# yeyupiaoling/MASR

Hardware: AMD Instinct MI355X
Metric: audio-seconds/sec (RTF^-1), conformer_streaming_fbank b32x10s, PCM->fbank->encoder->ctc_greedy->text (higher is better)
Workload: dtype f32; 1 GPU; configs[1]: conformer.yml streaming fbank, batch=32 synthetic 16 kHz 10 s utterances per GPU, ctc_greedy, random-init weights V=4233; global_batch=32, parallelism=dp1, world_size_observed=1, backend=none

## Files before the change

masr_amd/csrc/common.h:

```cpp
#pragma once
#include <hip/hip_runtime.h>
#include <stdint.h>

#include "lm_scorer.h"

#ifndef MASR_EXPERIMENTS
#define MASR_EXPERIMENTS 0
#endif

typedef float f32x4 __attribute__((ext_vector_type(4)));
typedef float f32x16 __attribute__((ext_vector_type(16)));

namespace masr {

struct LdsAttr {
    size_t granted[32] = {};
};
void ensure_dynamic_lds(const void* fn, size_t bytes, LdsAttr& st);
void note_launch_error(const char* what, hipError_t e);

#ifdef __HIPCC__
struct SeqRow {
    int b, t;
};
__device__ __forceinline__ SeqRow seq_row(int b0, int t0, int T, int lr) {
    SeqRow r{b0, t0 + lr};
    while (r.t >= T) {
        r.t -= T;
        ++r.b;
    }
    return r;
}

__device__ __forceinline__ float wave_sum_dpp(float v) {
#define MASR_DPP_F(x, ctrl, rows) \
    __builtin_bit_cast(float, __builtin_amdgcn_update_dpp(0, __builtin_bit_cast(int, (x)), (ctrl), (rows), 0xf, false))
    v += MASR_DPP_F(v, 0x111, 0xf);
    v += MASR_DPP_F(v, 0x112, 0xf);
    v += MASR_DPP_F(v, 0x114, 0xf);
    v += MASR_DPP_F(v, 0x118, 0xf);
    v += MASR_DPP_F(v, 0x142, 0xa);
    v += MASR_DPP_F(v, 0x143, 0xc);
#undef MASR_DPP_F
    return __builtin_bit_cast(float, __builtin_amdgcn_readlane(__builtin_bit_cast(int, v), 63));
}
#endif


enum GemmAct { ACT_NONE = 0, ACT_RELU = 1, ACT_SILU = 2 };
enum GemmAMode { A_PLAIN = 0, A_CONV2 = 1 };
enum GemmEpi { EPI_STD = 0, EPI_GLU = 1, EPI_SPLITK = 2 };

struct GemmArgs {
    const float* A;
    const float* W;
    const float* bias;
    float* C;
    const float* R;
    const int* lens;
    int M, N, K;
    int lda, ldc, ldr;
    int act;
    float alpha;
    int mask_tp;
    int bias_after_alpha;
    int T1, F1, T2, F2, Cc;
    int nsplit, ksplit;
    int skip_rps, skip_div;
};

void launch_gemm(const GemmArgs& a, int amode, int epi, hipStream_t s);
void set_conv2_mid_fill(int pct);
void set_gemm_waves(int n);
void launch_gemm_splitk(const GemmArgs& a, float* partial, int nsplit, hipStream_t s, int amode = A_PLAIN);
#if MASR_EXPERIMENTS
bool launch_gemm_bf16x3(const GemmArgs& a, int amode, hipStream_t s);
void set_gemm_bf16x3_waves(int n);
size_t ffn_x3_packed_elems(int dff);
void set_ffn_x3_rotation(int on);
void launch_pack_ffn_x3(const float* w1, const float* w2, unsigned short* p1, unsigned short* p2, int dff, hipStream_t s);
bool launch_ffn_x3(float* x, const float* lnw, const float* lnb, const unsigned short* p1, const float* b1,
                   const unsigned short* p2, const float* b2, int M, int dff, float eps, float scale, hipStream_t s);
#else
inline bool launch_gemm_bf16x3(const GemmArgs&, int, hipStream_t) { return false; }
inline void set_gemm_bf16x3_waves(int) {}
inline size_t ffn_x3_packed_elems(int) { return 0; }
inline void set_ffn_x3_rotation(int) {}
inline void launch_pack_ffn_x3(const float*, const float*, unsigned short*, unsigned short*, int, hipStream_t) {}
inline bool launch_ffn_x3(float*, const float*, const float*, const unsigned short*, const float*, const unsigned short*, const float*,
                          int, int, float, float, hipStream_t) { return false; }
#endif

void launch_layernorm(const float* x, const float* w, const float* b, float* y, int M, float eps,
                      int seq_t, int pad, const int* lens, hipStream_t s);
void set_conv1_nt(int on);
void launch_conv1(const float* feats, const float* mean, const float* istd, const float* w9c, const float* bias,
                  float* out, int B, int T, int F, int C, hipStream_t s);
void launch_dwconv_ln_silu(const float* g, const float* wkc, const float* bias, const float* lnw, const float* lnb,
                           float* out, int nseq, int Tq, int ktaps, float eps, hipStream_t s, const float* gconst = nullptr);
void launch_glu_const(const float* bias512, float* out256, hipStream_t s);
void launch_queue_spin(long long ticks, hipStream_t s);
void launch_queue_nop(hipStream_t s);
void launch_dwconv_bn_silu(const float* g, const float* wkc, const float* bias, const float* scale, const float* shift,
                           float* out, int nseq, int Tq, int ktaps, hipStream_t s, const float* gconst = nullptr);
void launch_dwconv_stride2_ln_silu(const float* g, const float* wkc, const float* bias, const float* lnw,
                                   const float* lnb, float* out, int nseq, int Tin, int ktaps, float eps, hipStream_t s);
void launch_avgpool2(const float* x, float* out, int B, int T, hipStream_t s);
void launch_time_reduce_dw(const float* x, const float* w5c, const float* bias, const int* lens, float* out, int B, int T,
                           int mstride, hipStream_t s);
void launch_recover_add(const float* saved, const float* y, float* x, int B, int T, int L, hipStream_t s);
void launch_softmax_argmax(float* logits, int M, int V, int ldv, int write_probs, int* idx, float* maxp, hipStream_t s);
void launch_ctc_collapse(const int* idx, const float* maxp, const int* nframes, int B, int Tp, int blank,
                         int* tokens, int* ntok, float* score, hipStream_t s);
struct PoolSeg {
    long src, dst;
    int n, pad_;
};
void launch_ctc_collapse_hist(const int* idx, const float* maxp, const int* nframes, const int* in_rows, int ld_in, int B, int Tp,
                              int blank, int* rows, hipStream_t s);
void launch_copy_segments(const float* src, float* dst, const float* src2, float* dst2, const PoolSeg* seg, int nseg,
                          int max_rows, int width, hipStream_t s);
void launch_ctc_collapse_rows(const int* idx, const float* maxp, const int* nframes, int B, int Tp, int blank, int* rows,
                              hipStream_t s);
void launch_topk_prune(const float* probs, int M, int V, int top_n, float cutoff_prob, int* out_idx, float* out_logp,
                       int* out_cnt, int blank, float* out_blank_lp, hipStream_t s);
void launch_argmax_rows(const float* probs, int M, int V, int* idx, float* maxp, hipStream_t s);
void launch_frame_counts(const int* nsamp, int B, int* nfr, int* nenc, int halve, hipStream_t s);
void launch_export_att(const float* cache, float* out, int L, int H, int cap, int t, int dk, hipStream_t s, int rate = 1,
                       int shift = 0);
struct PlaneCopy { const float* src_k; const float* src_v; float* dst_k; float* dst_v; };
void launch_kv_append_planar(const PlaneCopy* pc, int n, int Tq, hipStream_t s);
void launch_export_cnn_layer(const float* cache, float* out, int used, int total, int d, hipStream_t s);
void launch_export_att_planar(const float* kplane, const float* vplane, float* out, int H, int t, int dk, hipStream_t s);
void launch_affine_rows(const float* x, const float* w, const float* b, float* y, int M, int seq_t, int pad, hipStream_t s);
void launch_export_cnn(const float* cache, float* out, int L, int pad, int d, hipStream_t s);

struct AttSeq;
enum RowGemmPro { RG_PRO_PLAIN = 0, RG_PRO_LN = 1, RG_PRO_LN_PAD = 2, RG_PRO_AFFINE = 3,
                  RG_PRO_HIST = 4, RG_PRO_DWCONV = 5 };
enum RowGemmEpi { RG_EPI_STORE = 0, RG_EPI_RESID = 1, RG_EPI_GLU = 2, RG_EPI_CTC = 3, RG_EPI_CHAIN = 4 };
struct RowGemmArgs {
    const float* A;
    const float* lnw;
    const float* lnb;
    const float* W;
    const float* Wp;
    const float* bias;
    float* C;
    const float* R;
    float* R2;
    const int* lens;
    int* out_idx;
    float* out_maxp;
    int M, N;
    int lda, ldc, ldr;
    float eps, alpha;
// ... 220 lines not shown
```

masr_amd/csrc/engine.hip:

```cpp
#include <math.h>
#include <stdio.h>
#include <stdlib.h>
#include <string.h>

#include <map>
#include <mutex>
#include <string>
#include <vector>

#include "../../include/masr_hip.h"
#include "common.h"

using namespace masr;
namespace masr {
int lm_device_view(masr_lm* lm, LmView* out);
bool lm_word_based(const masr_lm* lm);
}
extern "C" const char* masr_lm_last_error(void);

static thread_local std::string g_err;
static int fail(const std::string& m) {
    g_err = m;
    return 1;
}
// ... 147 lines not shown
    int kin;
};

struct HostTensor {
    std::vector<float> v;
    std::vector<int64_t> shape;
};

struct Stream {
    bool open = false;
    int offset = 0;
    int offset_r = 0;
    int cap = 0;
    int history = -1;
    int cache_t1 = 0;
    int first_half = 0;
    DevBuf att;
    DevBuf cnn;
    DevBuf cnn2;
};

struct GBeam {
    bool open = false, started = false;
    int beam = 0, blank = 0, cap = 0;
    DevBuf pool, state;
    masr_lm* lm = nullptr;
    float alpha = 0.f, beta = 0.f;
};

enum ProfKind { PROF_NONE = 0, PROF_GEMM = 1, PROF_FFN1 = 2, PROF_CONV2 = 3, PROF_ATT = 4, PROF_FBANK = 5,
                PROF_FFN_TAIL = 6, PROF_FFN_HEAD = 7 };

}

struct EngineWs {
    DevBuf gx, rnn_out, hstate, cstate, ds2_lens;
    PinnedStage stage;
    DevBuf qplanes, attp, cnnptrs, ffpart;
    DevBuf fb_scratch;
    DevBuf x1, x2, x, ln, hid, qkv, att, lnpad, glu, dwo, logits, feats, enc, idx, maxp, attseq, gain, nframes, lens, xsave,
        xred, xh;
    void release_all() {
        for (DevBuf* b : {&gx, &rnn_out, &hstate, &cstate, &ds2_lens, &qplanes, &attp, &cnnptrs, &ffpart, &fb_scratch, &x1, &x2, &x,
                          &ln, &hid, &qkv, &att, &lnpad, &glu, &dwo, &logits, &feats, &enc, &idx, &maxp, &attseq, &gain, &nframes,
                          &lens, &xsave, &xred, &xh})
            b->release();
        stage.release();
    }
};

static int clear_sync(void* p, int value, size_t n) {
    HIPCHK(hipMemset(p, value, n));
    HIPCHK(hipStreamSynchronize(nullptr));
    return 0;
}

struct masr_engine : EngineWs {
    masr_config cfg;
    EngineWs parked[MASR_LANES];
    int lane = 0;
    hipEvent_t pack_ev = nullptr;
    void* pack_stream = nullptr;
    bool pack_pending = false;
    bool finalized = false;
    std::map<std::string, HostTensor> host;
    std::vector<void*> owned;
    float *cmvn_mean = nullptr, *cmvn_istd = nullptr, *conv1_w = nullptr, *conv1_b = nullptr, *conv2_w = nullptr,
          *conv2_b = nullptr, *embed_w = nullptr, *embed_b = nullptr, *after_w = nullptr, *after_b = nullptr,
          *ctc_w = nullptr, *ctc_b = nullptr, *pe = nullptr;
    std::vector<LayerW> layers;
    std::vector<SqLayerW> sq_layers;
    std::vector<Ds2LayerW> ds2_layers;
    std::vector<GBeam> gbeams;
    DevBuf beam_pool, beam_state;
    std::map<void*, std::pair<DevBuf, DevBuf>> beam_ws;
    std::map<void*, DevBuf> ms_ws;
    int skip_padding = 7;
    void* beam_first_stream = nullptr;
    bool beam_first_set = false;
    std::map<const float*, std::pair<DevBuf, DevBuf>> ffn_packed;
    std::map<const float*, std::pair<DevBuf, DevBuf>> ffn_dual_packed;
    std::map<const float*, std::pair<DevBuf, DevBuf>> x3_packed;
    std::map<const float*, std::pair<DevBuf, DevBuf>> ffn16_packed;
    long long* beam_prof = nullptr;
    float *preln_w = nullptr, *preln_b = nullptr, *tr_dw_w = nullptr, *tr_dw_b = nullptr, *tr_pw_w = nullptr,
          *tr_pw_b = nullptr, *rec_w = nullptr, *rec_b = nullptr;
    int reduce_idx = -1, recover_idx = -1;
    int stride_idx = -1, n_group_layers = 0, group_size = 3;
    bool conv_bn = false;
    float *window = nullptr, *melwt = nullptr, *tw512 = nullptr, *twr4 = nullptr;
    FbankTables fbank_tables() const { return FbankTables{window, melwt, tw512, twr4, mel_lo}; }
    int* mel_lo = nullptr;
    float *dct = nullptr, *lifter = nullptr;
    int dct_ceps = 0;
    double *lin_win = nullptr, *lin_tw = nullptr;
    double lin_scale = 0.0;
    std::vector<Stream> streams;
    int prof_kind = 0;
    int prof_stride = 1, prof_seen = 0;
    std::vector<std::pair<hipEvent_t, hipEvent_t>> prof_events;
    size_t prof_used = 0;
    double prof_flops = 0.0;
};

namespace {

template <class T>
int upload(masr_engine* e, const std::vector<T>& v, T** out) {
    void* p = nullptr;
    HIPCHK(hipMalloc(&p, std::max<size_t>(v.size(), 1) * sizeof(T)));
    HIPCHK(hipMemcpy(p, v.data(), v.size() * sizeof(T), hipMemcpyHostToDevice));
    e->owned.push_back(p);
    *out = reinterpret_cast<T*>(p);
    return 0;
}

int get(masr_engine* e, const std::string& name, std::vector<int64_t> shape, const HostTensor** out) {
    auto it = e->host.find(name);
    if (it == e->host.end()) return fail("missing tensor: " + name);
    int64_t want = 1, have = 1;
    for (auto s : shape) want *= s;
    for (auto s : it->second.shape) have *= s;
    if (want != have)
        return fail("tensor " + name + ": expected " + std::to_string(want) + " elements, got " + std::to_string(have));
    *out = &it->second;
    return 0;
}

int up(masr_engine* e, const std::string& name, std::vector<int64_t> shape, float** out) {
    const HostTensor* t;
    CHK(get(e, name, shape, &t));
    return upload(e, t->v, out);
}

struct ProfScope {
    masr_engine* e;
    hipStream_t s;
    bool on;
    ProfScope(masr_engine* e_, hipStream_t s_, int kind, double flops) : e(e_), s(s_) {
        on = e->prof_kind != 0 && (e->prof_kind == kind || (e->prof_kind == PROF_GEMM && (kind == PROF_FFN1 || kind == PROF_CONV2 || kind == PROF_FFN_TAIL || kind == PROF_FFN_HEAD)));
        if (on && e->prof_stride > 1) on = (e->prof_seen++ % e->prof_stride) == 0;
        if (!on) return;
        if (e->prof_used == e->prof_events.size()) {
            hipEvent_t a, b;
            hipEventCreate(&a);
            hipEventCreate(&b);
            e->prof_events.push_back({a, b});
        }
        hipEventRecord(e->prof_events[e->prof_used].first, s);
        e->prof_flops += flops;
    }
    ~ProfScope() {
        if (!on) return;
        hipEventRecord(e->prof_events[e->prof_used].second, s);
        e->prof_used++;
    }
};

struct CallGuard {
    masr_engine* e;
    hipStream_t s;
    size_t n0;
    static size_t packed_count(const masr_engine* e) {
        return e->ffn_packed.size() + e->ffn_dual_packed.size() + e->x3_packed.size() + e->ffn16_packed.size();
    }
    CallGuard(masr_engine* e_, hipStream_t s_) : e(e_), s(s_), n0(packed_count(e_)) {
        if (!e->pack_pending) return;
        if (hipEventQuery(e->pack_ev) == hipSuccess) {
            e->pack_pending = false;
        } else {
            (void)hipGetLastError();
            if ((void*)s != e->pack_stream) (void)hipStreamWaitEvent(s, e->pack_ev, 0);
        }
    }
    ~CallGuard() {
        if (packed_count(e) == n0) return;
        if (!e->pack_ev && hipEventCreateWithFlags(&e->pack_ev, hipEventDisableTiming) != hipSuccess) return;
        if (hipEventRecord(e->pack_ev, s) == hipSuccess) {
            e->pack_stream = (void*)s;
            e->pack_pending = true;
        }
    }
};

static int g_ffn_dual = 0;
static int g_ffn_packed = 2;
static int g_ffn16 = 1;
static int g_bf16x3 = 0;

void gemm(masr_engine* e, hipStream_t s, const float* A, int lda, const float* W, const float* bias, float* C, int ldc,
          int M, int N, int K, int act, float alpha, const float* R, int ldr, int kind = PROF_GEMM,
          const int* lens = nullptr, int mask_tp = 0) {
    GemmArgs a{};
    a.A = A; a.W = W; a.bias = bias; a.C = C; a.R = R; a.lens = lens;
    a.M = M; a.N = N; a.K = K; a.lda = lda; a.ldc = ldc; a.ldr = ldr;
    a.act = act; a.alpha = alpha; a.mask_tp = mask_tp;
    ProfScope ps(e, s, kind, 2.0 * M * (double)N * K);
    if (g_bf16x3 && launch_gemm_bf16x3(a, A_PLAIN, s)) return;
    launch_gemm(a, A_PLAIN, EPI_STD, s);
}

static int g_rowgemm_packed = 1;
const float* packed_rows_of(masr_engine* e, const float* W, int N, hipStream_t s) {
    auto it = e->ffn_packed.find(W);
    if (it == e->ffn_packed.end()) {
        const int Np = (N + 255) / 256 * 256;
        std::pair<DevBuf, DevBuf> pk;
        if (pk.first.ensure((size_t)Np * 256 * sizeof(float))) return nullptr;
        launch_pack_rows_pc(W, pk.first.as<float>(), Np, s, N);
        it = e->ffn_packed.emplace(W, pk).first;
    }
    return it->second.first.as<float>();
}

int packed_ffn_of(masr_engine* e, const float* w1, const float* w2, hipStream_t s, const float** p1, const float** p2) {
    const int d = e->cfg.d_model;
    auto it = e->ffn_packed.find(w1);
    if (it == e->ffn_packed.end()) {
        std::pair<DevBuf, DevBuf> pk;
        CHK(pk.first.ensure((size_t)e->cfg.d_ff * d * sizeof(float)));
        CHK(pk.second.ensure((size_t)e->cfg.d_ff * d * sizeof(float)));
        launch_pack_ffn_pc(w1, w2, pk.first.as<float>(), pk.second.as<float>(), e->cfg.d_ff, s);
        it = e->ffn_packed.emplace(w1, pk).first;
    }
    *p1 = it->second.first.as<float>();
    *p2 = it->second.second.as<float>();
    return 0;
}
static bool sqz_stage_supported(const masr_engine* e) {
    const int K = e->cfg.cnn_kernel;
    return e->cfg.d_model == 256 && e->cfg.d_ff % 128 == 0 && e->cfg.d_ff >= 256 && (K == 31 || K == 15);
}

void rowgemm(masr_engine* e, hipStream_t s, int pro, int epi, const float* A, int lda, const float* lnw,
             const float* lnb, const float* W, const float* bias, float* C, int ldc, int M, int N, const float* R,
             int ldr, float alpha, const int* lens, int mask_tp, int seq_t, int pad, int* out_idx, float* out_maxp,
             int kind = PROF_GEMM, int mstride = 4, int out_seq_t = 0, int out_pad_l = 0, int out_pad_tot = 0,
             int plane_cols = 0, long plane_stride = 0, int a_seq_t = 0, int a_seq_stride = 0, const AttSeq* kv_seqs = nullptr,
             int kv_tq = 0) {
    RowGemmArgs a{};
    a.A = A; a.lda = lda; a.lnw = lnw; a.lnb = lnb; a.W = W; a.bias = bias; a.C = C; a.ldc = ldc; a.M = M; a.N = N;
    a.R = R; a.ldr = ldr; a.alpha = alpha; a.lens = lens; a.mask_tp = mask_tp; a.seq_t = seq_t; a.pad = pad;
    a.out_idx = out_idx; a.out_maxp = out_maxp; a.eps = 1e-5f; a.mstride = mstride;
    a.out_seq_t = out_seq_t; a.out_pad_l = out_pad_l; a.out_pad_tot = out_pad_tot;
    a.plane_cols = plane_cols; a.plane_stride = plane_stride; a.a_seq_t = a_seq_t; a.a_seq_stride = a_seq_stride;
    a.kv_seqs = kv_seqs; a.kv_tq = kv_tq;
    if (g_rowgemm_packed && M >= 112 * 32 && pro != RG_PRO_HIST && pro != RG_PRO_DWCONV && (epi == RG_EPI_CTC || N % 256 == 0))
        a.Wp = packed_rows_of(e, W, N, s);
    ProfScope ps(e, s, kind, 2.0 * M * (double)N * 256);
    launch_rowgemm(a, pro, epi, s);
}

}

namespace {
int build_fbank_tables(masr_engine* e) {
    {
        std::vector<float> win(400), tw512(2 * 257), melw((size_t)80 * 257, 0.f);
        std::vector<int> lo(80), hi(80);
        for (int i = 0; i < 400; ++i) {
            const double hann = 0.5 - 0.5 * cos(2.0 * M_PI * i / 399.0);
            win[i] = (float)pow(hann, 0.85);
        }
        for (int k = 0; k <= 256; ++k) {
            tw512[2 * k] = (float)cos(-2.0 * M_PI * k / 512.0);
            tw512[2 * k + 1] = (float)sin(-2.0 * M_PI * k / 512.0);
        }
        const double mel_low = 1127.0 * log(1.0 + 20.0 / 700.0), mel_high = 1127.0 * log(1.0 + 8000.0 / 700.0);
        const float delta = (float)((mel_high - mel_low) / 81.0), mlow = (float)mel_low;
        for (int m = 0; m < 80; ++m) {
// ... 117 lines not shown
    if (cfg->model_kind < 0 || cfg->model_kind > 3)
        return fail("model_kind must be 0 (conformer), 1 (squeezeformer, non-streaming), 2 (efficient_conformer) or 3 (deepspeech2)");
    if (cfg->n_mels < 7 || cfg->n_mels > 512) return fail("input feature size (n_mels) must be in [7, 512]");
    if (cfg->model_kind == 3) {
        if (cfg->d_model != 1024) return fail("deepspeech2: the LSTM step kernel is specialised for rnn_size=1024");
        if (cfg->num_blocks <= 0) return fail("deepspeech2: num_rnn_layers must be positive");
    } else if (cfg->d_model != 256 || cfg->heads != 4) {
        return fail("kernels are specialised for d_model=256, heads=4");
    } else if (cfg->d_ff % 128) {
        return fail("unsupported d_ff");
    }
    if (cfg->model_kind == 3) {
    } else if (cfg->model_kind == 0 || cfg->model_kind == 2) {
        if (cfg->cnn_kernel != 15) return fail("conformer: cnn_module_kernel must be 15");
    } else {
        if (cfg->cnn_kernel != 31) return fail("squeezeformer: cnn_module_kernel must be 31");
    }
    int ndev = 0;
    HIPCHK(hipGetDeviceCount(&ndev));
    if (ndev <= 0) return fail("no HIP device");
    HIPCHK(hipSetDevice(cfg->device_id));
    {
        SideStreams* ss = nullptr;
        if (side_streams_of(cfg->device_id, &ss)) return 1;
    }
    masr_engine* e = new masr_engine();
    e->cfg = *cfg;
    if (e->cfg.max_pos <= 0) e->cfg.max_pos = 5000;
    e->reduce_idx = cfg->model_kind == 1 ? cfg->reserved[0] : -1;
    e->conv_bn = cfg->model_kind == 0 && cfg->reserved[0] == 1;
    e->recover_idx = cfg->model_kind == 1 ? cfg->reserved[1] : -1;
    if (cfg->model_kind == 2) {
        e->stride_idx = cfg->reserved[0];
        e->n_group_layers = cfg->reserved[1];
        e->group_size = cfg->reserved[2];
        if (e->group_size != 3) { delete e; return fail("efficient_conformer: group_size must be 3"); }
    }
    if (build_fbank_tables(e)) {
        masr_destroy(e);
        return 1;
    }
    *out = e;
    return 0;
}

void masr_destroy(masr_engine* e) {
    if (!e) return;
    for (void* p : e->owned) (void)hipFree(p);
    e->release_all();
    for (auto& w : e->parked) w.release_all();
    e->beam_pool.release();
    e->beam_state.release();
    if (e->pack_ev) (void)hipEventDestroy(e->pack_ev);
    for (auto& s : e->streams) {
        s.att.release();
        s.cnn.release();
        s.cnn2.release();
    }
    for (auto& g : e->gbeams) {
        g.pool.release();
        g.state.release();
    }
    for (auto& kv : e->beam_ws) {
        kv.second.first.release();
        kv.second.second.release();
    }
    for (auto& kv : e->ms_ws) kv.second.release();
    for (auto& kv : e->x3_packed) {
        kv.second.first.release();
        kv.second.second.release();
    }
    for (auto& kv : e->ffn_packed) {
        kv.second.first.release();
        kv.second.second.release();
    }
    for (auto& kv : e->ffn_dual_packed) {
        kv.second.first.release();
        kv.second.second.release();
    }
    for (auto& kv : e->ffn16_packed) {
        kv.second.first.release();
        kv.second.second.release();
    }
    for (auto& ev : e->prof_events) {
        (void)hipEventDestroy(ev.first);
        (void)hipEventDestroy(ev.second);
    }
    delete e;
}

static void drop_packed_weights(masr_engine* e) {
    if (e->ffn_packed.empty() && e->ffn_dual_packed.empty() && e->x3_packed.empty() && e->ffn16_packed.empty()) return;
    (void)hipSetDevice(e->cfg.device_id);
    (void)hipDeviceSynchronize();
    for (auto* m : {&e->ffn_packed, &e->ffn_dual_packed, &e->x3_packed, &e->ffn16_packed}) {
        for (auto& kv : *m) {
            kv.second.first.release();
            kv.second.second.release();
        }
        m->clear();
    }
}

int masr_load_tensor(masr_engine* e, const char* name, const float* host, const int64_t* shape, int32_t ndim) {
    if (!e || !name || !host) return fail("null argument");
    std::string n(name);
    if (n.rfind("encoder.", 0) != 0 && n.rfind("ctc.", 0) != 0 && n.rfind("decoder.ctc_lo.", 0) != 0 && n != "__pos_table__")
        return 0;
    drop_packed_weights(e);
    HostTensor t;
    int64_t cnt = 1;
    for (int i = 0; i < ndim; ++i) {
        t.shape.push_back(shape[i]);
        cnt *= shape[i];
    }
    t.v.assign(host, host + cnt);
    e->host[n] = std::move(t);
    e->finalized = false;
    return 0;
}

static int finalize_squeezeformer(masr_engine* e, hipStream_t s);
static int finalize_ds2(masr_engine* e);
static int enc_dim(const masr_engine* e) {
    return e->cfg.model_kind == 3 ? e->cfg.d_model * (e->cfg.causal ? 1 : 2) : e->cfg.d_model;
}
static int layer_kernel(const masr_engine* e, int i) {
    return (e->cfg.model_kind == 2 && e->stride_idx >= 0 && i > e->stride_idx) ? e->cfg.cnn_kernel / 2 : e->cfg.cnn_kernel;
}
static bool layer_grouped(const masr_engine* e, int i) { return e->cfg.model_kind == 2 && i < e->n_group_layers; }

int masr_finalize(masr_engine* e, void* stream) {
    if (!e) return fail("null engine");
    if (e->cfg.model_kind == 1) return finalize_squeezeformer(e, (hipStream_t)stream);
    if (e->cfg.model_kind == 3) return finalize_ds2(e);
    hipStream_t s = (hipStream_t)stream;
    HIPCHK(hipSetDevice(e->cfg.device_id));
    const int d = e->cfg.d_model, dff = e->cfg.d_ff, L = e->cfg.num_blocks, V = e->cfg.vocab_size, F = e->cfg.n_mels;
    const int F1 = (F - 1) / 2, F2 = (F1 - 1) / 2, K = e->cfg.cnn_kernel, H = e->cfg.heads, dk = d / H;
    const HostTensor* t;
    CHK(up(e, "encoder.global_cmvn.mean", {F}, &e->cmvn_mean));
    CHK(up(e, "encoder.global_cmvn.istd", {F}, &e->cmvn_istd));
    {
        CHK(get(e, "encoder.embed.conv.0.weight", {d, 1, 3, 3}, &t));
        std::vector<float> w(9 * d);
        for (int c = 0; c < d; ++c)
            for (int k = 0; k < 9; ++k) w[k * d + c] = t->v[c * 9 + k];
        CHK(upload(e, w, &e->conv1_w));
        CHK(up(e, "encoder.embed.conv.0.bias", {d}, &e->conv1_b));
    }
    {
        CHK(get(e, "encoder.embed.conv.2.weight", {d, d, 3, 3}, &t));
        std::vector<float> w((size_t)d * 9 * d);
        for (int co = 0; co < d; ++co)
            for (int ci = 0; ci < d; ++ci)
                for (int k = 0; k < 9; ++k)
                    w[(size_t)co * 9 * d + (size_t)(ci / 32) * 9 * 32 + k * 32 + ci % 32] = t->v[((size_t)co * d + ci) * 9 + k];
        CHK(upload(e, w, &e->conv2_w));
        CHK(up(e, "encoder.embed.conv.2.bias", {d}, &e->conv2_b));
    }
    {
        CHK(get(e, "encoder.embed.out.0.weight", {d, (int64_t)d * F2}, &t));
        std::vector<float> w((size_t)d * d * F2);
        for (int o = 0; o < d; ++o)
            for (int c = 0; c < d; ++c)
                for (int f = 0; f < F2; ++f) w[(size_t)o * d * F2 + f * d + c] = t->v[(size_t)o * d * F2 + c * F2 + f];
        CHK(upload(e, w, &e->embed_w));
        CHK(up(e, "encoder.embed.out.0.bias", {d}, &e->embed_b));
    }
    {
        auto it = e->host.find("__pos_table__");
        if (it != e->host.end()) {
            if ((int64_t)it->second.v.size() != (int64_t)e->cfg.max_pos * d) return fail("__pos_table__ has wrong size");
            CHK(upload(e, it->second.v, &e->pe));
        } else {
            std::vector<float> pe((size_t)e->cfg.max_pos * d);
            for (int i = 0; i < d; i += 2) {
                const float div = expf((float)i * (float)(-(log(10000.0) / d)));
// ... 259 lines not shown
            auto it = e->ffn16_packed.find(W);
            if (it == e->ffn16_packed.end()) {
                std::pair<DevBuf, DevBuf> pk;
                CHK(pk.first.ensure((size_t)N * d * sizeof(float)));
                launch_pack_rows16(W, pk.first.as<float>(), N, s);
                it = e->ffn16_packed.emplace(W, pk).first;
            }
            *out = it->second.first.as<float>();
            return 0;
        };
        auto it = e->ffn16_packed.find(w1);
        if (it == e->ffn16_packed.end()) {
            std::pair<DevBuf, DevBuf> pk;
            CHK(pk.first.ensure((size_t)dff * d * sizeof(float)));
            CHK(pk.second.ensure((size_t)dff * d * sizeof(float)));
            launch_pack_ffn16(w1, w2, pk.first.as<float>(), pk.second.as<float>(), dff, s);
            it = e->ffn16_packed.emplace(w1, pk).first;
        }
        if (want_tail) {
            ptail = *tail;
            CHK(p16(tail->W, tail->N, &ptail.W));
        }
        if (want_head) {
            phead = *head;
            CHK(p16(head->W, d, &phead.W));
        }
        const int done = launch_ffn16(e->x.as<float>(), lnw, lnb, it->second.first.as<float>(), b1, it->second.second.as<float>(), b2, M,
                                      dff, 1e-5f, scale, s, want_tail ? &ptail : nullptr, want_head ? &phead : nullptr);
        if (done < 0) return fail("ffn(): the 16-row FFN kernel rejected the launch");
        if (want_head && done != 4) return fail("ffn(): head stage was not launched");
        if (tail_done) *tail_done = done == 2;
        if (post_y) launch_layernorm(e->x.as<float>(), post_w, post_b, post_y, M, 1e-5f, 0, 0, nullptr, s);
        return 0;
    }
    if (packed && want_tail && tail->N % 256 == 0) {
        ptail = *tail;
        CHK(packed_rows(tail->W, tail->N, &ptail.W));
        tail = &ptail;
    }
    if (packed && want_head) {
        phead = *head;
        CHK(packed_rows(head->W, d, &phead.W));
        if (split_head) {
            CHK(e->xh.ensure((size_t)M * d * sizeof(float)));
            phead.xout = e->xh.as<float>();
        }
        head = &phead;
    }
    const int done = launch_ffn_fused(e->x.as<float>(), lnw, lnb, kw1, b1, kw2, b2, M, dff, 1e-5f, scale, affine,
                                      nsplit > 1 ? e->ffpart.as<float>() : nullptr, nsplit, s, post_y ? &post : nullptr,
                                      want_tail ? tail : nullptr, want_head ? head : nullptr, packed);
    if (done < 0) return fail("ffn(): launch rejected");
    if (want_head && !(done & 4)) return fail("ffn(): head stage was not launched");
    if (tail_done) *tail_done = done == 2;
    if (post_y && !(done & 1)) launch_layernorm(e->x.as<float>(), post_w, post_b, post_y, M, 1e-5f, 0, 0, nullptr, s);
    return 0;
}

static int g_hot_weights = 0;
static int g_embed_split = 1;
int embed(masr_engine* e, hipStream_t s, const float* feats, int nseq, int T, int* Tq_out, const int* skip_lens = nullptr) {
    const int d = e->cfg.d_model, F = e->cfg.n_mels, F1 = (F - 1) / 2, F2 = (F1 - 1) / 2;
    const int T1 = (T - 1) / 2, Tq = (T1 - 1) / 2;
    if (T < 7 || Tq <= 0) return fail("input too short for Conv2dSubsampling4 (need >= 7 frames)");
    const int M = nseq * Tq;
    CHK(e->x1.ensure((size_t)nseq * T1 * F1 * d * sizeof(float)));
    CHK(e->x2.ensure((size_t)M * F2 * d * sizeof(float)));
    CHK(e->x.ensure((size_t)M * d * sizeof(float)));
    launch_conv1(feats, e->cmvn_mean, e->cmvn_istd, e->conv1_w, e->conv1_b, e->x1.as<float>(), nseq, T, F, d, s);
    {
        GemmArgs a{};
        a.A = e->x1.as<float>(); a.W = e->conv2_w; a.bias = e->conv2_b; a.C = e->x2.as<float>();
        a.M = M * F2; a.N = d; a.K = 9 * d; a.ldc = d; a.act = ACT_RELU; a.alpha = 1.f;
        a.T1 = T1; a.F1 = F1; a.T2 = Tq; a.F2 = F2; a.Cc = d;
        if (skip_lens) { a.lens = skip_lens; a.skip_rps = Tq * F2; a.skip_div = F2; }
        ProfScope ps(e, s, PROF_CONV2, 2.0 * a.M * (double)a.N * a.K);
        const int tiles = ((a.M + 63) / 64) * ((a.N + 63) / 64);
        if (g_bf16x3 && tiles >= 640 && launch_gemm_bf16x3(a, A_CONV2, s)) {
        } else if (tiles < 640) {
            const int nsplit = std::min(8, std::max(2, 1280 / tiles));
            CHK(e->ffpart.ensure((size_t)nsplit * a.M * a.N * sizeof(float)));
            launch_gemm_splitk(a, e->ffpart.as<float>(), nsplit, s, A_CONV2);
        } else {
            launch_gemm(a, A_CONV2, EPI_STD, s);
        }
    }
    {
        GemmArgs a{};
        a.A = e->x2.as<float>(); a.lda = F2 * d; a.W = e->embed_w; a.bias = e->embed_b; a.C = e->x.as<float>(); a.ldc = d;
        a.M = M; a.N = d; a.K = F2 * d; a.act = ACT_NONE; a.alpha = sqrtf((float)d);
        a.bias_after_alpha = e->cfg.model_kind == 1 ? 1 : 0;
        if (skip_lens) { a.lens = skip_lens; a.skip_rps = Tq; a.skip_div = 1; }
        ProfScope ps(e, s, PROF_GEMM, 2.0 * M * (double)d * F2 * d);
        const int tiles = ((M + 63) / 64) * ((d + 63) / 64);
        const long wide = (long)((M + 63) / 64) * ((d + 127) / 128);
        const long t128 = (long)((M + 127) / 128) * ((d + 127) / 128);
        if (g_bf16x3 && tiles >= 128 && launch_gemm_bf16x3(a, A_PLAIN, s)) {
        } else if (g_embed_split && tiles >= 128 && t128 >= 100 && t128 <= 128) {
            CHK(e->ffpart.ensure((size_t)4 * M * d * sizeof(float)));
            launch_gemm_splitk(a, e->ffpart.as<float>(), 4, s);
        } else if (g_embed_split && tiles >= 128 && wide >= 200 && wide <= 320) {
            CHK(e->ffpart.ensure((size_t)2 * M * d * sizeof(float)));
            launch_gemm_splitk(a, e->ffpart.as<float>(), 2, s);
        } else if (tiles < 128) {
            const int nsplit = std::min(F2 * d / 32, std::max(2, 256 / tiles));
            CHK(e->ffpart.ensure((size_t)nsplit * M * d * sizeof(float)));
            launch_gemm_splitk(a, e->ffpart.as<float>(), nsplit, s);
        } else {
            launch_gemm(a, A_PLAIN, EPI_STD, s);
        }
    }
    *Tq_out = Tq;
    return 0;
}

int ensure_layer_ws(masr_engine* e, int nseq, int Tq) {
    const int d = e->cfg.d_model, pad = e->cfg.cnn_kernel - 1;
    const size_t M = (size_t)nseq * Tq;
    CHK(e->ln.ensure(M * d * sizeof(float)));
    CHK(e->qkv.ensure(M * 3 * d * sizeof(float)));
    CHK(e->att.ensure(M * d * sizeof(float)));
    CHK(e->lnpad.ensure((size_t)nseq * (Tq + pad) * d * sizeof(float)));
    CHK(e->glu.ensure((size_t)nseq * (Tq + pad) * d * sizeof(float)));
    CHK(e->dwo.ensure(M * d * sizeof(float)));
    return 0;
}

int conv_module(masr_engine* e, hipStream_t s, const LayerW& w, const EncodeCtx& c, bool hist, int K = 0, int mstride = 4,
                bool pw1_done = false, bool pw2_later = false) {
    if (K <= 0) K = e->cfg.cnn_kernel;
    const int d = e->cfg.d_model, pad = K - 1;
    const int M = c.nseq * c.Tq, Mp = c.nseq * (c.Tq + pad);
    float* x = e->x.as<float>();
    if (pw1_done) {
    } else if (hist) {
        launch_layernorm(x, w.ln_conv_w, w.ln_conv_b, e->lnpad.as<float>(), M, 1e-5f, c.Tq, pad, c.lens, s);
        rowgemm(e, s, RG_PRO_PLAIN, RG_EPI_GLU, e->lnpad.as<float>(), d, nullptr, nullptr, w.pw1_w, w.pw1_b,
                e->glu.as<float>(), d, Mp, 2 * d, nullptr, 0, 1.f, nullptr, 0, 0, 0, nullptr, nullptr);
    } else {
        rowgemm(e, s, RG_PRO_LN_PAD, RG_EPI_GLU, x, d, w.ln_conv_w, w.ln_conv_b, w.pw1_w, w.pw1_b, e->glu.as<float>(), d,
                M, 2 * d, nullptr, 0, 1.f, c.lens, 0, c.Tq, 0, nullptr, nullptr, PROF_GEMM, mstride, c.Tq,
                e->cfg.causal ? pad : pad / 2, pad);
    }
    if (pw2_later) return 0;
    const float* gconst = (hist || !e->cfg.causal) ? nullptr : w.gconst;
    {
        RowGemmArgs a{};
        a.A = e->glu.as<float>(); a.lda = d; a.lnw = w.cln_w; a.lnb = w.cln_b; a.dw_w = w.dw_w; a.dw_b = w.dw_b; a.gconst = gconst;
        a.W = w.pw2_w; a.bias = w.pw2_b; a.C = x; a.ldc = d; a.R = x; a.ldr = d; a.M = M; a.N = d; a.alpha = 1.f; a.eps = 1e-5f;
        a.mstride = mstride; a.seq_t = c.Tq; a.pad = pad; a.lens = c.lens; a.mask_tp = c.lens ? c.Tq : 0;
        ProfScope ps(e, s, PROF_GEMM, 2.0 * M * (double)d * d);
        if (!e->conv_bn && g_few_rows_path && launch_rowgemm(a, RG_PRO_DWCONV, RG_EPI_RESID, s)) return 0;
    }
    if (e->conv_bn)
        launch_dwconv_bn_silu(e->glu.as<float>(), w.dw_w, w.dw_b, w.cln_w, w.cln_b, e->dwo.as<float>(), c.nseq, c.Tq, K, s, gconst);
    else
        launch_dwconv_ln_silu(e->glu.as<float>(), w.dw_w, w.dw_b, w.cln_w, w.cln_b, e->dwo.as<float>(), c.nseq, c.Tq, K,
                              1e-5f, s, gconst);
    rowgemm(e, s, RG_PRO_PLAIN, RG_EPI_RESID, e->dwo.as<float>(), d, nullptr, nullptr, w.pw2_w, w.pw2_b, x, d, M, d, x, d,
            1.f, c.lens, c.lens ? c.Tq : 0, 0, 0, nullptr, nullptr, PROF_GEMM, mstride);
    return 0;
}

int conv_module_stream(masr_engine* e, hipStream_t s, const LayerW& w, int n, int Tq, float* const* cache_rd,
                       float* const* cache_wr, int K, bool pw2_later = false) {
    const int d = e->cfg.d_model, pad = K - 1, M = n * Tq, Mp = n * (Tq + pad);
// ... 1592 lines not shown
    } else if (cnn_dev) {
        launch_export_cnn(st->cnn.as<float>(), cnn_dev, L, pad, d, s);
    }
    LAUNCHCHK();
    return 0;
}


int masr_op_layernorm(masr_engine* e, const float* x_dev, const float* w_dev, const float* b_dev, float* y_dev,
                      int32_t M, float eps, void* stream) {
    if (!e) return fail("null engine");
    ENTER(e);
    launch_layernorm(x_dev, w_dev, b_dev, y_dev, M, eps, 0, 0, nullptr, (hipStream_t)stream);
    LAUNCHCHK();
    return 0;
}

int masr_op_gemm(masr_engine* e, const float* a_dev, const float* w_dev, const float* bias_dev, const float* res_dev,
                 float* c_dev, int32_t M, int32_t N, int32_t K, int32_t act, float alpha, void* stream) {
    if (!e) return fail("null engine");
    ENTER(e);
    CallGuard call_guard(e, (hipStream_t)stream);
    if (K % 32) return fail("K must be a multiple of 32");
    gemm(e, (hipStream_t)stream, a_dev, K, w_dev, bias_dev, c_dev, N, M, N, K, act, alpha, res_dev, N);
    LAUNCHCHK();
    return 0;
}

int masr_select_lane(masr_engine* e, int32_t lane) {
    if (!e) return fail("null engine");
    if (lane < 0 || lane >= MASR_LANES) return fail("masr_select_lane: lane must be in [0, " + std::to_string(MASR_LANES) + ")");
    if (lane == e->lane) return 0;
    EngineWs& active = *e;
    e->parked[e->lane] = active;
    active = e->parked[lane];
    e->parked[lane] = EngineWs();
    e->lane = lane;
    return 0;
}

int masr_side_stream(masr_engine* e, int32_t kind, void** stream_out) {
    if (!e || !stream_out) return fail("null argument");
    if (kind < 0 || kind >= MASR_SIDE_STREAMS)
        return fail("masr_side_stream: kind must be 0 / 1 (prefix search), 2 (preparation), 3 (copy) or 4 (second encoder lane)");
    SideStreams* ss = nullptr;
    if (side_streams_of(e->cfg.device_id, &ss)) return 1;
    *stream_out = (void*)ss->s[kind];
    return 0;
}

int masr_debug_set(masr_engine* e, int32_t key, int32_t value) {
    if (!e) return fail("null engine");
#if !MASR_EXPERIMENTS
    if (value != 0 && (key == 20 || key == 21 || key == 22 || key == 24 || key == 30 || key == 34 || key == 35))
        return fail("masr_debug_set: this key selects an experimental kernel that is not in this build (MASR_BUILD_EXPERIMENTS=1)");
#endif
    if (key == 1) set_ffn_variant(value);
    else if (key == 5) g_no_chain = value;
    else if (key == 6) set_rowgemm_small(value);
    else if (key == 7) set_attention_fewq(value);
    else if (key == 14) set_attention_fold(value);
    else if (key == 15) g_embed_split = value;
    else if (key == 19) g_hot_weights = value;
    else if (key == 20) g_bf16x3 = value;
    else if (key == 21) set_gemm_bf16x3_waves(value);
    else if (key == 22) set_ffn_x3_rotation(value);
    else if (key == 23) g_ffn_packed = value;
    else if (key == 24) g_ffn_dual = value;
    else if (key == 25) g_rowgemm_packed = value;
    else if (key == 26) set_attention_grouped_fold(value);
    else if (key == 27) g_ctc_fused_blocks = value;
    else if (key == 28) set_attention_fewq_wgs(value);
    else if (key == 29) g_few_rows_path = value;
    else if (key == 30) g_split_head = value;
    else if (key == 31) g_efficient_fused = value;
    else if (key == 32) g_beam_lm_cache = value;
    else if (key == 33) set_conv2_mid_fill(value);
    else if (key == 34) g_attn_chain = value;
    else if (key == 35) g_ffn_coop = value;
    else if (key == 36) g_sqz_fused_blocks = value;
    else if (key == 37) g_beam_narrow = value;
    else if (key == 38) e->skip_padding = value;
    else if (key == 39) g_ffn16 = value;
    else if (key == 17) set_gemm_waves(value);
    else if (key == 18) set_conv1_nt(value);
    else if (key == 16) { e->prof_stride = value > 1 ? value : 1; e->prof_seen = 0; }
    else if (key == 8) g_no_ffn_tail = value;
    else if (key == 9) g_no_ffn_head = value;
    else if (key == 12) set_rowgemm_small_blocks(value);
    else if (key == 13) g_ffn_split_blocks = value;
    else if (key == 2) {
        if (value) {
            if (!e->beam_prof) {
                void* p = nullptr;
                HIPCHK(hipMalloc(&p, 16 * sizeof(long long)));
                e->owned.push_back(p);
                e->beam_prof = (long long*)p;
            }
        } else if (e->beam_prof) {
            long long h[16];
            HIPCHK(hipMemcpy(h, e->beam_prof, sizeof(h), hipMemcpyDeviceToHost));
            fprintf(stderr, "beam phases (cycles, last workgroup): setup+hash %lld  extensions %lld  prefixes+count %lld  select %lld  compact %lld\n",
                    h[0], h[1], h[2], h[3], h[4]);
            fprintf(stderr, "  narrow step (%lld frames): tables+candidates %lld  hash+contexts %lld  children+scorer table %lld  extensions %lld  "
                    "prefixes+select %lld  scan %lld  survivors %lld  new prefixes %lld\n", h[5], h[6], h[7], h[8], h[9], h[10], h[11], h[12], h[13]);
            if (h[15] > 0) fprintf(stderr, "  wide step (%lld frames): %.1f distinct scorer contexts per frame\n", h[15], (double)h[14] / (double)h[15]);
            e->beam_prof = nullptr;
        }
    }
    else return fail("unknown debug key");
    return 0;
}

int masr_profile_select(masr_engine* e, int32_t kind) {
    if (!e) return fail("null engine");
    e->prof_kind = kind;
    return 0;
}

int masr_profile_read(masr_engine* e, double* total_ms, int64_t* launches, double* flops, int32_t reset) {
    if (!e) return fail("null engine");
    ENTER(e);
    double tot = 0.0;
    for (size_t i = 0; i < e->prof_used; ++i) {
        HIPCHK(hipEventSynchronize(e->prof_events[i].second));
        float ms = 0.f;
        HIPCHK(hipEventElapsedTime(&ms, e->prof_events[i].first, e->prof_events[i].second));
        tot += ms;
    }
    if (total_ms) *total_ms = tot;
    if (launches) *launches = (int64_t)e->prof_used;
    if (flops) *flops = e->prof_flops;
    if (reset) {
        e->prof_used = 0;
        e->prof_flops = 0.0;
    }
    return 0;
}

}
```

masr_amd/csrc/gemm_f32.hip:

```cpp
#include "common.h"

namespace masr {

static constexpr int BK = 32;
static constexpr int LDP = 36;

__device__ __forceinline__ float silu_f(float x) { return x / (1.0f + expf(-x)); }
__device__ __forceinline__ float sigmoid_f(float x) { return 1.0f / (1.0f + expf(-x)); }

template <int BM, int BN, int WM, int WN, int AMODE, int EPI>
__global__ __launch_bounds__(64 * WM * WN) void gemm_f32_kernel(GemmArgs p) {
    static_assert(WM * WN == 4 || WM * WN == 8, "4 or 8 waves");
    constexpr int NT = 64 * WM * WN;
    constexpr int RPP = NT / 8;
    constexpr int TM = BM / WM / 32;
    constexpr int TN = BN / WN / 32;
    constexpr int AL = BM / RPP;
    constexpr int WL = BN / RPP;
    extern __shared__ __align__(16) float smem[];
    float* As = smem;
    float* Ws = smem + 2 * BM * LDP;

    const int tid = threadIdx.x;
    const int lane = tid & 63;
// ... 81 lines not shown
    const int KT = EPI == EPI_SPLITK ? min(kt_lo + p.ksplit, p.K / BK) : p.K / BK;
    load_slab(kt_lo);
    store_slab(0);
    __syncthreads();

    const int frow = lane & 31;
    const int fcol = (lane >> 5) * 4;
    for (int kt = kt_lo; kt < KT; ++kt) {
        const int buf = (kt - kt_lo) & 1;
        if (kt + 1 < KT) load_slab(kt + 1);
        __builtin_amdgcn_sched_barrier(0);
        const float* Ab = &As[(buf * BM + wm * (BM / WM) + frow) * LDP + fcol];
        const float* Wb = &Ws[(buf * BN + wn * (BN / WN) + frow) * LDP + fcol];
#pragma unroll
        for (int g = 0; g < BK / 8; ++g) {
            f32x4 af[TM], wf[TN];
#pragma unroll
            for (int m = 0; m < TM; ++m) af[m] = *reinterpret_cast<const f32x4*>(Ab + m * 32 * LDP + g * 8);
#pragma unroll
            for (int n = 0; n < TN; ++n) wf[n] = *reinterpret_cast<const f32x4*>(Wb + n * 32 * LDP + g * 8);
#pragma unroll
            for (int s = 0; s < 4; ++s)
#pragma unroll
                for (int m = 0; m < TM; ++m)
#pragma unroll
                    for (int n = 0; n < TN; ++n)
                        acc[m][n] = __builtin_amdgcn_mfma_f32_32x32x2f32(af[m][s], wf[n][s], acc[m][n], 0, 0, 0);
        }
        __builtin_amdgcn_sched_barrier(0);
        if (kt + 1 < KT) store_slab(buf ^ 1);
        __syncthreads();
    }

    const int ccol = lane & 31;
    const int rbase = 4 * (lane >> 5);
    if (EPI == EPI_SPLITK) {
        float* cp = p.C + (size_t)blockIdx.y * p.M * p.ldc;
#pragma unroll
        for (int n = 0; n < TN; ++n) {
            const int col = bn + wn * (BN / WN) + n * 32 + ccol;
            if (col >= p.N) continue;
#pragma unroll
            for (int m = 0; m < TM; ++m)
#pragma unroll
                for (int r = 0; r < 16; ++r) {
                    const int row = bm + wm * (BM / WM) + m * 32 + (r & 3) + 8 * (r >> 2) + rbase;
                    if (row < p.M) cp[(size_t)row * p.ldc + col] = acc[m][n][r];
                }
        }
    }
    if (EPI == EPI_STD) {
#pragma unroll
        for (int n = 0; n < TN; ++n) {
            const int col = bn + wn * (BN / WN) + n * 32 + ccol;
            if (col >= p.N) continue;
            const float bv = p.bias ? p.bias[col] : 0.f;
#pragma unroll
            for (int m = 0; m < TM; ++m) {
                float res[16];
#pragma unroll
                for (int r = 0; r < 16; ++r) {
                    const int row = min(bm + wm * (BM / WM) + m * 32 + (r & 3) + 8 * (r >> 2) + rbase, p.M - 1);
                    res[r] = p.R ? p.R[(size_t)row * p.ldr + col] : 0.f;
                }
#pragma unroll
                for (int r = 0; r < 16; ++r) {
                    const int row = bm + wm * (BM / WM) + m * 32 + (r & 3) + 8 * (r >> 2) + rbase;
                    float v = acc[m][n][r] + (p.bias_after_alpha ? 0.f : bv);
                    if (p.act == ACT_RELU) v = fmaxf(v, 0.f);
                    else if (p.act == ACT_SILU) v = silu_f(v);
                    if (p.mask_tp > 0) {
                        const int rc = min(row, p.M - 1);
                        const int b = rc / p.mask_tp, t = rc - b * p.mask_tp;
                        if (4 * t >= p.lens[b]) v = 0.f;
                    }
                    v = res[r] + v * p.alpha + (p.bias_after_alpha ? bv : 0.f);
                    if (row < p.M) p.C[(size_t)row * p.ldc + col] = v;
                }
            }
        }
    }
}

static int g_gemm_waves = 8;
static int g_conv2_mid_fill = 50;
void set_conv2_mid_fill(int pct) { g_conv2_mid_fill = pct; }
void set_gemm_waves(int n) { g_gemm_waves = n; }

template <int BM, int BN, int WM, int WN, int AMODE, int EPI>
static void launch_t(const GemmArgs& a, hipStream_t s) {
    const int nbm = (a.M + BM - 1) / BM, nbn = (a.N + BN - 1) / BN;
    const size_t lds = (size_t)2 * (BM + BN) * LDP * sizeof(float);
    auto k = gemm_f32_kernel<BM, BN, WM, WN, AMODE, EPI>;
    static LdsAttr attr;
    ensure_dynamic_lds(reinterpret_cast<const void*>(k), lds, attr);
    hipLaunchKernelGGL(k, dim3(nbm * nbn, EPI == EPI_SPLITK ? a.nsplit : 1), dim3(64 * WM * WN), lds, s, a);
}

__global__ __launch_bounds__(256) void splitk_reduce_kernel(GemmArgs p, const float* __restrict__ partial, float* out) {
    const size_t i = (size_t)blockIdx.x * 256 + threadIdx.x;
    if (i >= (size_t)p.M * p.N) return;
    const int row = (int)(i / p.N), col = (int)(i - (size_t)row * p.N);
    float acc = 0.f;
    for (int sp = 0; sp < p.nsplit; ++sp) acc += partial[((size_t)sp * p.M + row) * p.N + col];
    const float bv = p.bias ? p.bias[col] : 0.f;
    float v = acc + (p.bias_after_alpha ? 0.f : bv);
    if (p.act == ACT_RELU) v = fmaxf(v, 0.f);
    else if (p.act == ACT_SILU) v = silu_f(v);
    const float r = p.R ? p.R[(size_t)row * p.ldr + col] : 0.f;
    out[(size_t)row * p.ldc + col] = r + v * p.alpha + (p.bias_after_alpha ? bv : 0.f);
}

void launch_gemm(const GemmArgs& a, int amode, int epi, hipStream_t s) {
    if (a.M <= 0 || a.N <= 0) return;
    if (amode == A_CONV2 && epi == EPI_SPLITK) {
        launch_t<64, 64, 2, 2, A_CONV2, EPI_SPLITK>(a, s);
        return;
    }
    if (amode == A_CONV2) {
        const long t128c = (long)((a.M + 127) / 128) * ((a.N + 127) / 128);
        const long rounds = (t128c + 511) / 512;
        const bool thin_tail = g_conv2_mid_fill > 0 && t128c >= 200 && t128c <= 1024 &&
                               (t128c - (rounds - 1) * 512) * 100 < (long)g_conv2_mid_fill * 512;
        if (t128c < 200) launch_t<64, 64, 2, 2, A_CONV2, EPI_STD>(a, s);
        else if (thin_tail) launch_t<64, 128, 2, 2, A_CONV2, EPI_STD>(a, s);
        else if (g_gemm_waves == 8) launch_t<128, 128, 2, 4, A_CONV2, EPI_STD>(a, s);
        else launch_t<128, 128, 2, 2, A_CONV2, EPI_STD>(a, s);
        return;
    }
    if (epi == EPI_SPLITK) {
        if (a.nsplit >= 4 && (long)((a.M + 127) / 128) * ((a.N + 127) / 128) >= 100) launch_t<128, 128, 2, 4, A_PLAIN, EPI_SPLITK>(a, s);
        else if ((long)((a.M + 63) / 64) * ((a.N + 127) / 128) >= 200) launch_t<64, 128, 2, 2, A_PLAIN, EPI_SPLITK>(a, s);
        else launch_t<64, 64, 2, 2, A_PLAIN, EPI_SPLITK>(a, s);
        return;
    }
    const long t128 = (long)((a.M + 127) / 128) * ((a.N + 127) / 128);
    const long t64 = (long)((a.M + 63) / 64) * ((a.N + 127) / 128);
    if (t128 >= 384) launch_t<128, 128, 2, 2, A_PLAIN, EPI_STD>(a, s);
    else if (t64 >= 200) launch_t<64, 128, 2, 2, A_PLAIN, EPI_STD>(a, s);
    else launch_t<64, 64, 2, 2, A_PLAIN, EPI_STD>(a, s);
}

void launch_gemm_splitk(const GemmArgs& a, float* partial, int nsplit, hipStream_t s, int amode) {
    if (a.M <= 0 || a.N <= 0) return;
    GemmArgs b = a;
    const int kts = a.K / BK;
    b.ksplit = (kts + nsplit - 1) / nsplit;
    b.nsplit = (kts + b.ksplit - 1) / b.ksplit;
    b.C = partial;
    b.ldc = a.N;
    launch_gemm(b, amode, EPI_SPLITK, s);
    GemmArgs r = a;
    r.nsplit = b.nsplit;
    hipLaunchKernelGGL(splitk_reduce_kernel, dim3((unsigned)(((size_t)a.M * a.N + 255) / 256)), dim3(256), 0, s, r, partial, a.C);
}

}
```

Measured before the change: 51250 audio-seconds/sec.

## Add row-block conv2 GEMM kernel streaming pre-packed weights from registers

Adds a dedicated conv2 subsampling GEMM kernel for N=256. Each 512-thread block covers 64 output rows and all 256 columns, with each wave owning 32 columns. Weights are repacked once into a per-lane fragment layout and streamed through a register ring via buffer loads, so only the A (im2col) tile goes through LDS with double buffering. The aim is to avoid redundant A loads across N-tiles and LDS traffic for weights; in exchange it adds a cached packed weight buffer and a one-time pack kernel, and only applies when the tile count is in the large, non-thin-tail range.

```diff
diff --git a/masr_amd/csrc/common.h b/masr_amd/csrc/common.h
--- a/masr_amd/csrc/common.h
+++ b/masr_amd/csrc/common.h
@@ -67,11 +67,13 @@
     int T1, F1, T2, F2, Cc;
     int nsplit, ksplit;
     int skip_rps, skip_div;
+    const float* Wp;
 };
 
 void launch_gemm(const GemmArgs& a, int amode, int epi, hipStream_t s);
 void set_conv2_mid_fill(int pct);
 void set_gemm_waves(int n);
+void launch_pack_conv2_rows(const float* w, float* p, int K, hipStream_t s);
 void launch_gemm_splitk(const GemmArgs& a, float* partial, int nsplit, hipStream_t s, int amode = A_PLAIN);
 #if MASR_EXPERIMENTS
 bool launch_gemm_bf16x3(const GemmArgs& a, int amode, hipStream_t s);
diff --git a/masr_amd/csrc/engine.hip b/masr_amd/csrc/engine.hip
--- a/masr_amd/csrc/engine.hip
+++ b/masr_amd/csrc/engine.hip
@@ -253,6 +253,7 @@
     std::map<const float*, std::pair<DevBuf, DevBuf>> ffn_dual_packed;
     std::map<const float*, std::pair<DevBuf, DevBuf>> x3_packed;
     std::map<const float*, std::pair<DevBuf, DevBuf>> ffn16_packed;
+    std::map<const float*, std::pair<DevBuf, DevBuf>> conv2_packed;
     long long* beam_prof = nullptr;
     float *preln_w = nullptr, *preln_b = nullptr, *tr_dw_w = nullptr, *tr_dw_b = nullptr, *tr_pw_w = nullptr,
           *tr_pw_b = nullptr, *rec_w = nullptr, *rec_b = nullptr;
@@ -333,7 +334,7 @@
     hipStream_t s;
     size_t n0;
     static size_t packed_count(const masr_engine* e) {
-        return e->ffn_packed.size() + e->ffn_dual_packed.size() + e->x3_packed.size() + e->ffn16_packed.size();
+        return e->ffn_packed.size() + e->ffn_dual_packed.size() + e->x3_packed.size() + e->ffn16_packed.size() + e->conv2_packed.size();
     }
     CallGuard(masr_engine* e_, hipStream_t s_) : e(e_), s(s_), n0(packed_count(e_)) {
         if (!e->pack_pending) return;
@@ -357,6 +358,7 @@
 static int g_ffn_dual = 0;
 static int g_ffn_packed = 2;
 static int g_ffn16 = 1;
+static int g_conv2_rows = 1;
 static int g_bf16x3 = 0;
 
 void gemm(masr_engine* e, hipStream_t s, const float* A, int lda, const float* W, const float* bias, float* C, int ldc,
@@ -640,6 +642,10 @@
         kv.second.first.release();
         kv.second.second.release();
     }
+    for (auto& kv : e->conv2_packed) {
+        kv.second.first.release();
+        kv.second.second.release();
+    }
     for (auto& ev : e->prof_events) {
         (void)hipEventDestroy(ev.first);
         (void)hipEventDestroy(ev.second);
@@ -648,10 +654,11 @@
 }
 
 static void drop_packed_weights(masr_engine* e) {
-    if (e->ffn_packed.empty() && e->ffn_dual_packed.empty() && e->x3_packed.empty() && e->ffn16_packed.empty()) return;
+    if (e->ffn_packed.empty() && e->ffn_dual_packed.empty() && e->x3_packed.empty() && e->ffn16_packed.empty() && e->conv2_packed.empty())
+        return;
     (void)hipSetDevice(e->cfg.device_id);
     (void)hipDeviceSynchronize();
-    for (auto* m : {&e->ffn_packed, &e->ffn_dual_packed, &e->x3_packed, &e->ffn16_packed}) {
+    for (auto* m : {&e->ffn_packed, &e->ffn_dual_packed, &e->x3_packed, &e->ffn16_packed, &e->conv2_packed}) {
         for (auto& kv : *m) {
             kv.second.first.release();
             kv.second.second.release();
@@ -1077,6 +1084,16 @@
             CHK(e->ffpart.ensure((size_t)nsplit * a.M * a.N * sizeof(float)));
             launch_gemm_splitk(a, e->ffpart.as<float>(), nsplit, s, A_CONV2);
         } else {
+            if (g_conv2_rows && a.N == 256) {
+                auto it = e->conv2_packed.find(e->conv2_w);
+                if (it == e->conv2_packed.end()) {
+                    std::pair<DevBuf, DevBuf> pk;
+                    CHK(pk.first.ensure((size_t)a.N * a.K * sizeof(float)));
+                    launch_pack_conv2_rows(e->conv2_w, pk.first.as<float>(), a.K, s);
+                    it = e->conv2_packed.emplace(e->conv2_w, pk).first;
+                }
+                a.Wp = it->second.first.as<float>();
+            }
             launch_gemm(a, A_CONV2, EPI_STD, s);
         }
     }
@@ -2835,6 +2852,7 @@
     else if (key == 37) g_beam_narrow = value;
     else if (key == 38) e->skip_padding = value;
     else if (key == 39) g_ffn16 = value;
+    else if (key == 40) g_conv2_rows = value;
     else if (key == 17) set_gemm_waves(value);
     else if (key == 18) set_conv1_nt(value);
     else if (key == 16) { e->prof_stride = value > 1 ? value : 1; e->prof_seen = 0; }
diff --git a/masr_amd/csrc/gemm_f32.hip b/masr_amd/csrc/gemm_f32.hip
--- a/masr_amd/csrc/gemm_f32.hip
+++ b/masr_amd/csrc/gemm_f32.hip
@@ -187,6 +187,147 @@
     }
 }
 
+static constexpr int RB_BM = 64;
+static constexpr int RB_N = 256;
+static constexpr int RB_RING = 8;
+
+__device__ __forceinline__ f32x4 rb_bufld(__amdgpu_buffer_rsrc_t rs, unsigned lane16, unsigned frag) {
+    return __builtin_bit_cast(f32x4, __builtin_amdgcn_raw_buffer_load_b128(rs, lane16, frag * 1024u, 0));
+}
+
+__global__ __launch_bounds__(512) __attribute__((amdgpu_waves_per_eu(4))) void conv2_rows_kernel(GemmArgs p) {
+    __shared__ __align__(16) float As[2][RB_BM * LDP];
+    const int tid = threadIdx.x, lane = tid & 63;
+    const int wave = __builtin_amdgcn_readfirstlane(tid >> 6);
+    const int nbm = (p.M + RB_BM - 1) / RB_BM;
+    int bid = blockIdx.x;
+    if (p.skip_rps <= 0) {
+        const int q = nbm / 8, r = nbm % 8, xcd = bid % 8, idx = bid / 8;
+        bid = (xcd < r ? xcd * (q + 1) : r * (q + 1) + (xcd - r) * q) + idx;
+    }
+    const int bm = bid * RB_BM;
+    if (p.skip_rps > 0 && p.lens) {
+        const int span = min(bm + RB_BM, p.M) - 1 - bm;
+        const int b0 = bm / p.skip_rps, r0 = bm - b0 * p.skip_rps;
+        if (r0 + span < p.skip_rps && 4 * (r0 / p.skip_div) >= p.lens[b0]) return;
+    }
+
+    const int lrow = tid >> 3, lc4 = (tid & 7) * 4;
+    const float* aptr;
+    const bool aok = bm + lrow < p.M;
+    {
+        const int mm = aok ? bm + lrow : 0;
+        const int f2 = mm % p.F2, bt = mm / p.F2, t2 = bt % p.T2, b = bt / p.T2;
+        aptr = p.A + (((size_t)b * p.T1 + 2 * t2) * p.F1 + 2 * f2) * p.Cc + lc4;
+    }
+    auto load_a = [&](int kt) -> f32x4 {
+        const int cb = kt / 9, pos = kt - 9 * cb;
+        const int kh = pos / 3, kw = pos - 3 * kh;
+        const size_t aoff = ((size_t)kh * p.F1 + kw) * p.Cc + (size_t)cb * BK;
+        return aok ? *reinterpret_cast<const f32x4*>(aptr + aoff) : f32x4{0.f, 0.f, 0.f, 0.f};
+    };
+    float* const adst = &As[0][lrow * LDP + lc4];
+
+    const int KT = p.K / BK;
+    const __amdgpu_buffer_rsrc_t wrs =
+        __builtin_amdgcn_make_buffer_rsrc(const_cast<float*>(p.Wp), 0, RB_N * p.K * (int)sizeof(float), 0x00020000);
+    const unsigned lane16 = lane * 16;
+    const unsigned wfrag0 = (unsigned)(wave * KT) * 4u;
+    auto bld = [&](int kt, int g) -> f32x4 { return rb_bufld(wrs, lane16, wfrag0 + (unsigned)min(kt, KT - 1) * 4u + g); };
+
+    f32x4 pre[RB_RING];
+#pragma unroll
+    for (int i = 0; i < RB_RING; ++i) pre[i] = bld(i >> 2, i & 3);
+    f32x16 acc[2];
+#pragma unroll
+    for (int m = 0; m < 2; ++m)
+#pragma unroll
+        for (int r = 0; r < 16; ++r) acc[m][r] = 0.f;
+
+    *reinterpret_cast<f32x4*>(adst) = load_a(0);
+    __syncthreads();
+
+    const int frow = lane & 31, fcol = (lane >> 5) * 4;
+    const float* afrag = &As[0][frow * LDP + fcol];
+    for (int kt0 = 0; kt0 < KT; kt0 += 2) {
+#pragma unroll
+        for (int j = 0; j < 2; ++j) {
+            const int kt = kt0 + j;
+            if (j == 1 && kt >= KT) break;
+            f32x4 areg;
+            if (kt + 1 < KT) areg = load_a(kt + 1);
+            const float* Ab = afrag + j * RB_BM * LDP;
+            f32x4 af[2] = {*reinterpret_cast<const f32x4*>(Ab), *reinterpret_cast<const f32x4*>(Ab + 32 * LDP)};
+            __builtin_amdgcn_sched_barrier(0);
+#pragma unroll
+            for (int g = 0; g < BK / 8; ++g) {
+                f32x4 an[2];
+                if (g + 1 < BK / 8) {
+                    an[0] = *reinterpret_cast<const f32x4*>(Ab + (g + 1) * 8);
+                    an[1] = *reinterpret_cast<const f32x4*>(Ab + 32 * LDP + (g + 1) * 8);
+                }
+                __builtin_amdgcn_sched_barrier(0);
+#pragma unroll
+                for (int s = 0; s < 4; ++s)
+#pragma unroll
+                    for (int m = 0; m < 2; ++m)
+                        acc[m] = __builtin_amdgcn_mfma_f32_32x32x2f32(af[m][s], pre[4 * j + g][s], acc[m], 0, 0, 0);
+                __builtin_amdgcn_sched_barrier(0);
+                pre[4 * j + g] = bld(kt + 2, g);
+                __builtin_amdgcn_sched_barrier(0);
+                if (g + 1 < BK / 8) {
+                    af[0] = an[0];
+                    af[1] = an[1];
+                }
+            }
+            if (kt + 1 < KT) *reinterpret_cast<f32x4*>(adst + (j ^ 1) * RB_BM * LDP) = areg;
+            __syncthreads();
+        }
+    }
+
+    const int ccol = lane & 31;
+    const int rbase = 4 * (lane >> 5);
+    const int col = wave * 32 + ccol;
+    const float bv = p.bias ? p.bias[col] : 0.f;
+#pragma unroll
+    for (int m = 0; m < 2; ++m) {
+        float res[16];
+#pragma unroll
+        for (int r = 0; r < 16; ++r) {
+            const int row = min(bm + m * 32 + (r & 3) + 8 * (r >> 2) + rbase, p.M - 1);
+            res[r] = p.R ? p.R[(size_t)row * p.ldr + col] : 0.f;
+        }
+#pragma unroll
+        for (int r = 0; r < 16; ++r) {
+            const int row = bm + m * 32 + (r & 3) + 8 * (r >> 2) + rbase;
+            float v = acc[m][r] + (p.bias_after_alpha ? 0.f : bv);
+            if (p.act == ACT_RELU) v = fmaxf(v, 0.f);
+            else if (p.act == ACT_SILU) v = silu_f(v);
+            if (p.mask_tp > 0) {
+                const int rc = min(row, p.M - 1);
+                const int b = rc / p.mask_tp, t = rc - b * p.mask_tp;
+                if (4 * t >= p.lens[b]) v = 0.f;
+            }
+            v = res[r] + v * p.alpha + (p.bias_after_alpha ? bv : 0.f);
+            if (row < p.M) p.C[(size_t)row * p.ldc + col] = v;
+        }
+    }
+}
+
+__global__ __launch_bounds__(256) void pack_conv2_rows_kernel(const float* __restrict__ w, float* __restrict__ p, int K) {
+    const size_t e = (size_t)blockIdx.x * 256 + threadIdx.x;
+    if (e >= (size_t)RB_N * K) return;
+    const int KT = K / BK;
+    const int q = (int)(e & 3), lane = (int)((e >> 2) & 63);
+    const size_t frag = e >> 8;
+    const int g = (int)(frag & 3), kt = (int)((frag >> 2) % KT), wave = (int)((frag >> 2) / KT);
+    p[e] = w[(size_t)(32 * wave + (lane & 31)) * K + kt * BK + 8 * g + 4 * (lane >> 5) + q];
+}
+void launch_pack_conv2_rows(const float* w, float* p, int K, hipStream_t s) {
+    const size_t n = (size_t)RB_N * K;
+    hipLaunchKernelGGL(pack_conv2_rows_kernel, dim3((unsigned)((n + 255) / 256)), dim3(256), 0, s, w, p, K);
+}
+
 static int g_gemm_waves = 8;
 static int g_conv2_mid_fill = 50;
 void set_conv2_mid_fill(int pct) { g_conv2_mid_fill = pct; }
@@ -229,6 +370,8 @@
                                (t128c - (rounds - 1) * 512) * 100 < (long)g_conv2_mid_fill * 512;
         if (t128c < 200) launch_t<64, 64, 2, 2, A_CONV2, EPI_STD>(a, s);
         else if (thin_tail) launch_t<64, 128, 2, 2, A_CONV2, EPI_STD>(a, s);
+        else if (a.Wp && a.N == RB_N && a.K % BK == 0)
+            hipLaunchKernelGGL(conv2_rows_kernel, dim3((unsigned)((a.M + RB_BM - 1) / RB_BM)), dim3(512), 0, s, a);
         else if (g_gemm_waves == 8) launch_t<128, 128, 2, 4, A_CONV2, EPI_STD>(a, s);
         else launch_t<128, 128, 2, 2, A_CONV2, EPI_STD>(a, s);
         return;
```

Result: faster. 52080 audio-seconds/sec (median of 6 runs) (+1.6%).
